# StarrickLiu/StarFlashAttention

Hardware: AMD Instinct MI355X
Metric: attention fwd TFLOPS/GPU (% MFMA peak), bf16 seqlen=4096 hdim=128 (higher is better)
Workload: dtype bf16; 1 GPU; prefill fwd causal, B=16 H=32 S=4096 D=128 per GPU (BASELINE.json configs[2]); batch-sharded, no collectives; global_batch=16, seq_len=4096, heads=32, head_dim=128, causal=True, parallelism=batch-shard x1

## Files before the change

starflashattention_amd/csrc/prefill_w4_kernel.hip:

```cpp
#include "prefill_w4_common.h"

namespace sfa {

namespace {

using namespace prefill;

namespace w4 {
typedef float f32x2 __attribute__((ext_vector_type(2)));

using namespace w4c;

constexpr int kRows = 256;
constexpr int kKeys = 64;
constexpr int kRing = 3;

template <int D> struct Img {
    static constexpr int RG = 512 * (D / 32);
    static constexpr int TILE = 8 * RG;
    static constexpr int K_BASE = 0;
    static constexpr int V_BASE = kRing * TILE;
    static constexpr int Q_BASE = 2 * kRing * TILE;
    static constexpr int TOTAL = Q_BASE + 4 * TILE;
};

#define SFA_AOWN \
    "a0", "a1", "a2", "a3", "a4", "a5", "a6", "a7", "a8", "a9", "a10", "a11", "a12", "a13", "a14", "a15", \
    "a16", "a17", "a18", "a19", "a20", "a21", "a22", "a23", "a24", "a25", "a26", "a27", "a28", "a29", "a30", "a31", \
    "a32", "a33", "a34", "a35", "a36", "a37", "a38", "a39", "a40", "a41", "a42", "a43", "a44", "a45", "a46", "a47", \
    "a48", "a49", "a50", "a51", "a52", "a53", "a54", "a55", "a56", "a57", "a58", "a59", "a60", "a61", "a62", "a63", \
    "a64", "a65", "a66", "a67", "a68", "a69", "a70", "a71", "a72", "a73", "a74", "a75", "a76", "a77", "a78", "a79", \
    "a80", "a81", "a82", "a83", "a84", "a85", "a86", "a87", "a88", "a89", "a90", "a91", "a92", "a93", "a94", "a95", \
    "a96", "a97", "a98", "a99", "a100", "a101", "a102", "a103", "a104", "a105", "a106", "a107", "a108", "a109", "a110", "a111", \
    "a112", "a113", "a114", "a115", "a116", "a117", "a118", "a119", "a120", "a121", "a122", "a123", "a124", "a125", "a126", "a127", \
    "a128", "a129", "a130", "a131", "a132", "a133", "a134", "a135", "a136", "a137", "a138", "a139", "a140", "a141", "a142", "a143", \
    "a144", "a145", "a146", "a147", "a148", "a149", "a150", "a151", "a152", "a153", "a154", "a155", "a156", "a157", "a158", "a159", \
    "a160", "a161", "a162", "a163", "a164", "a165", "a166", "a167", "a168", "a169", "a170", "a171", "a172", "a173", "a174", "a175", \
    "a176", "a177", "a178", "a179", "a180", "a181", "a182", "a183", "a184", "a185", "a186", "a187", "a188", "a189", "a190", "a191"
constexpr int o_reg(int q, int d) { return 16 * (4 * q + d); }
constexpr int q_reg(int q, int ks) { return 128 + 4 * (8 * q + ks); }

template <class Tr, int QB>
__device__ __forceinline__ void own_qk_first(f32x16 &s, typename Tr::mfma_vec k) {
    if constexpr (Tr::id == 1) asm volatile("v_mfma_f32_32x32x16_bf16 %0, %1, a[%c2:%c3], 0" : "=&v"(s) : "v"(k), "n"(QB), "n"(QB + 3) : SFA_AOWN);
    else asm volatile("v_mfma_f32_32x32x16_f16 %0, %1, a[%c2:%c3], 0" : "=&v"(s) : "v"(k), "n"(QB), "n"(QB + 3) : SFA_AOWN);
}
template <class Tr, int QB>
__device__ __forceinline__ void own_qk_first_c(f32x16 &s, typename Tr::mfma_vec k, const f32x16 &c) {
    if constexpr (Tr::id == 1) asm volatile("s_nop 1\n\tv_mfma_f32_32x32x16_bf16 %0, %1, a[%c2:%c3], %4" : "=&v"(s) : "v"(k), "n"(QB), "n"(QB + 3), "v"(c) : SFA_AOWN);
    else asm volatile("s_nop 1\n\tv_mfma_f32_32x32x16_f16 %0, %1, a[%c2:%c3], %4" : "=&v"(s) : "v"(k), "n"(QB), "n"(QB + 3), "v"(c) : SFA_AOWN);
}
template <class Tr, int QB>
__device__ __forceinline__ void own_qk(f32x16 &s, typename Tr::mfma_vec k) {
    if constexpr (Tr::id == 1) asm volatile("v_mfma_f32_32x32x16_bf16 %0, %1, a[%c2:%c3], %0" : "+v"(s) : "v"(k), "n"(QB), "n"(QB + 3) : SFA_AOWN);
    else asm volatile("v_mfma_f32_32x32x16_f16 %0, %1, a[%c2:%c3], %0" : "+v"(s) : "v"(k), "n"(QB), "n"(QB + 3) : SFA_AOWN);
}
template <class Tr, int OB>
__device__ __forceinline__ void own_pv(typename Tr::mfma_vec v, typename Tr::mfma_vec pfrag) {
    if constexpr (Tr::id == 1) asm volatile("v_mfma_f32_32x32x16_bf16 a[%c2:%c3], %0, %1, a[%c2:%c3]" :: "v"(v), "v"(pfrag), "n"(OB), "n"(OB + 15) : SFA_AOWN);
    else asm volatile("v_mfma_f32_32x32x16_f16 a[%c2:%c3], %0, %1, a[%c2:%c3]" :: "v"(v), "v"(pfrag), "n"(OB), "n"(OB + 15) : SFA_AOWN);
}
template <class Tr, int OB>
__device__ __forceinline__ void own_zero(typename Tr::mfma_vec z) {
    if constexpr (Tr::id == 1) asm volatile("s_nop 1\n\tv_mfma_f32_32x32x16_bf16 a[%c1:%c2], %0, %0, 0" :: "v"(z), "n"(OB), "n"(OB + 15) : SFA_AOWN);
    else asm volatile("s_nop 1\n\tv_mfma_f32_32x32x16_f16 a[%c1:%c2], %0, %0, 0" :: "v"(z), "n"(OB), "n"(OB + 15) : SFA_AOWN);
}
__device__ __forceinline__ void own_settle() { asm volatile("s_nop 15\n\ts_nop 15" ::: SFA_AOWN); }
template <int R>
__device__ __forceinline__ float own_read() {
    float x;
    asm volatile("v_accvgpr_read_b32 %0, a%c1" : "=v"(x) : "n"(R) : SFA_AOWN);
    return x;
}
template <int R>
__device__ __forceinline__ void own_scale(float f) {
    float t;
    asm volatile("v_accvgpr_read_b32 %0, a%c2\n\tv_mul_f32 %0, %0, %1\n\tv_accvgpr_write_b32 a%c2, %0" : "=&v"(t) : "v"(f), "n"(R) : SFA_AOWN);
}

template <int D>
struct Acc {
    float msc[2];
    float lsum[2];
    float alpha[2];
    uint32_t pk[2][8];
    f32x16 cinit[2];
};
struct Fin {
    float lsum[2];
    float msc[2];
};

template <int D>
__device__ __forceinline__ void rescale_o(int q, float alpha) {
    own_settle();
    static_for<16 * (D / 32)>([&](auto ic) {
        constexpr int r = decltype(ic)::value;
        if (q == 0) own_scale<o_reg(0, 0) + r>(alpha);
        else own_scale<o_reg(1, 0) + r>(alpha);
    });
    asm volatile("s_nop 1" ::: SFA_AOWN);
}

constexpr int kLead = 8;
constexpr float kNoKey = -1.0e30f;

__device__ __forceinline__ constexpr int el_q(int i) { return (i >> 3) & 1; }
__device__ __forceinline__ constexpr int el_r(int i) { return 8 * (i >> 4) + (i & 7); }

template <class Tr, int ORD, int I>
__device__ __forceinline__ void st_f(f32x16 (&s)[2], const float (&msc)[2], float c2) {
    if constexpr (ORD != 6 && I >= 0 && I < 32)
        asm volatile("v_fma_f32 %0, %0, %1, -%2" : "+v"(s[el_q(I)][el_r(I)]) : "s"(c2), "v"(msc[el_q(I)]));
}
template <int I>
__device__ __forceinline__ void st_x(f32x16 (&s)[2]) {
    if constexpr (I >= 0 && I < 32) asm volatile("v_exp_f32 %0, %0" : "+v"(s[el_q(I)][el_r(I)]));
}
template <class Tr, int I>
__device__ __forceinline__ void st_a(f32x16 (&s)[2], float (&lsum)[2], uint32_t (&pk)[2][8]) {
    if constexpr (I >= 0 && I < 32) {
        constexpr int q = el_q(I), r = el_r(I);
        asm volatile("v_add_f32 %0, %0, %1" : "+v"(lsum[q]) : "v"(s[q][r]));
        if constexpr (I & 1) {
            if constexpr (Tr::id == 1) asm volatile("v_cvt_pk_bf16_f32 %0, %1, %2" : "=v"(pk[q][r >> 1]) : "v"(s[q][r - 1]), "v"(s[q][r]));
            else asm volatile("v_cvt_pk_f16_f32 %0, %1, %2" : "=v"(pk[q][r >> 1]) : "v"(s[q][r - 1]), "v"(s[q][r]));
        }
    }
}
template <class Tr, int D, int ORD>
__device__ __forceinline__ void decide(Acc<D> &acc, int q, f32x16 &s, float mxl, float c2, int &pend) {
    if (ORD == 6) {
        if (__any(mxl > kThr)) {
            const float d = fmaxf(half_max(mxl), 0.f);
            const float al = fast_exp2(-d);
            acc.msc[q] += d;
            acc.lsum[q] *= al;
            acc.alpha[q] = al;
            pend = 1;
#pragma unroll
            for (int r = 0; r < 16; ++r) { s[r] -= d; acc.cinit[q][r] = -acc.msc[q]; }
        }
        return;
    }
    if (__any(__builtin_fmaf(mxl, c2, -kThr) > acc.msc[q])) {
        const float mx = half_max(mxl) * c2;
        const float mnew = fmaxf(acc.msc[q], mx);
        const float al = fast_exp2(acc.msc[q] - mnew);
        acc.msc[q] = mnew;
        acc.lsum[q] *= al;
        acc.alpha[q] = al;
        pend = 1;
    }
}
template <class Tr, int D, int ORD>
__device__ __forceinline__ void fresh_start(Acc<D> &acc, Fin &fin, int q, f32x16 &s, float mxl, float c2) {
    fin.lsum[q] = acc.lsum[q];
    fin.msc[q] = acc.msc[q];
    const float mx = half_max(mxl);
    acc.lsum[q] = 0.f;
    if (ORD == 6) {
        const float m0 = (mx == ninf()) ? 0.f : mx;
        acc.msc[q] = m0;
#pragma unroll
        for (int r = 0; r < 16; ++r) { s[r] -= m0; acc.cinit[q][r] = -m0; }
    } else {
        acc.msc[q] = fmaxf(mx * c2, kNoKey);
    }
}

template <int D>
__device__ __forceinline__ void apply_pending(Acc<D> &acc, int &pend) {
    if (pend) {
#pragma unroll
        for (int q = 0; q < 2; ++q) { rescale_o<D>(q, acc.alpha[q]); acc.alpha[q] = 1.0f; }
        pend = 0;
    }
}

__device__ __forceinline__ int lane_now() {
    int l = __builtin_amdgcn_mbcnt_hi(~0u, __builtin_amdgcn_mbcnt_lo(~0u, 0u));
    asm volatile("" : "+v"(l));
    return l;
}
__device__ __forceinline__ f32x16 mask_tuple(int kbase, int qrow0, int klast) {
    const int l = lane_now();
    const int room = min(klast, qrow0 + (l & 31)) - kbase - 4 * (l >> 5);
    const float ni = ninf();
    float c[16];
    asm volatile(
        "v_cmp_gt_i32_e32 vcc, 0, %16\n\tv_cndmask_b32_e32 %0, 0, %17, vcc\n\t"
        "v_cmp_gt_i32_e32 vcc, 1, %16\n\tv_cndmask_b32_e32 %1, 0, %17, vcc\n\t"
        "v_cmp_gt_i32_e32 vcc, 2, %16\n\tv_cndmask_b32_e32 %2, 0, %17, vcc\n\t"
        "v_cmp_gt_i32_e32 vcc, 3, %16\n\tv_cndmask_b32_e32 %3, 0, %17, vcc\n\t"
        "v_cmp_gt_i32_e32 vcc, 8, %16\n\tv_cndmask_b32_e32 %4, 0, %17, vcc\n\t"
        "v_cmp_gt_i32_e32 vcc, 9, %16\n\tv_cndmask_b32_e32 %5, 0, %17, vcc\n\t"
        "v_cmp_gt_i32_e32 vcc, 10, %16\n\tv_cndmask_b32_e32 %6, 0, %17, vcc\n\t"
        "v_cmp_gt_i32_e32 vcc, 11, %16\n\tv_cndmask_b32_e32 %7, 0, %17, vcc\n\t"
        "v_cmp_gt_i32_e32 vcc, 16, %16\n\tv_cndmask_b32_e32 %8, 0, %17, vcc\n\t"
        "v_cmp_gt_i32_e32 vcc, 17, %16\n\tv_cndmask_b32_e32 %9, 0, %17, vcc\n\t"
        "v_cmp_gt_i32_e32 vcc, 18, %16\n\tv_cndmask_b32_e32 %10, 0, %17, vcc\n\t"
        "v_cmp_gt_i32_e32 vcc, 19, %16\n\tv_cndmask_b32_e32 %11, 0, %17, vcc\n\t"
        "v_cmp_gt_i32_e32 vcc, 24, %16\n\tv_cndmask_b32_e32 %12, 0, %17, vcc\n\t"
        "v_cmp_gt_i32_e32 vcc, 25, %16\n\tv_cndmask_b32_e32 %13, 0, %17, vcc\n\t"
        "v_cmp_gt_i32_e32 vcc, 26, %16\n\tv_cndmask_b32_e32 %14, 0, %17, vcc\n\t"
        "v_cmp_gt_i32_e32 vcc, 27, %16\n\tv_cndmask_b32_e32 %15, 0, %17, vcc"
        : "=&v"(c[0]), "=&v"(c[1]), "=&v"(c[2]), "=&v"(c[3]), "=&v"(c[4]), "=&v"(c[5]), "=&v"(c[6]), "=&v"(c[7]), "=&v"(c[8]),
          "=&v"(c[9]), "=&v"(c[10]), "=&v"(c[11]), "=&v"(c[12]), "=&v"(c[13]), "=&v"(c[14]), "=&v"(c[15])
        : "v"(room), "v"(ni)
        : "vcc");
    f32x16 cm;
#pragma unroll
    for (int r = 0; r < 16; ++r) cm[r] = c[r];
    return cm;
}

template <class Tr, int D, int ORD, int HO, int PH, int NEW, int OLD, int MK, class Hook = NoHook>
__device__ __forceinline__ void hstep(const lds_char *lds, unsigned k_e, unsigned v_e, int vbuf, int kbuf_pref,
                                      f32x16 (&sN)[2], f32x16 (&sO)[2],
                                      Acc<D> &acc, Fin &fin, int &pend, float c2, int mask_n, int kbase_n, int qbase_n,
                                      int klast, const f32x16 &diag0, const f32x16 &ninf16, typename Tr::mfma_vec (&kpre)[D / 16],
                                      const Hook &hook = Hook()) {
    using Vec = typename Tr::mfma_vec;
    constexpr int NKS = D / 16, NDB = D / 32;
    constexpr int RG = Img<D>::RG;
// ... 350 lines not shown
        const unsigned qvoff1 = (unsigned)(qr8 + 8) * rowb + 64u * qsub + 16u * (qslot ^ (2 + (qr8 >> 2)));
        const unsigned long long base = (unsigned long long)(uintptr_t)(a->q + b * a->qs0 + h * a->qs1) + (unsigned long long)row0 * rowb;
        u32x4s srd;
        srd[0] = (unsigned)base;
        srd[1] = (unsigned)(base >> 32) & 0xffffu;
        srd[2] = row0 < a->Sq ? (unsigned)(a->Sq - 1 - row0) * rowb + 2u * D : 0u;
        srd[3] = 0x00020000u;
        const unsigned dst = lds0 + L::Q_BASE + wave * L::TILE;
#pragma unroll
        for (int rg = 0; rg < 8; ++rg)
#pragma unroll
            for (int j = 0; j < NJ; ++j)
                dma_piece(dst + rg * L::RG + 1024 * j, (rg & 1) ? qvoff1 : qvoff0, srd, 128u * j + 16u * (rg >> 1) * rowb);
        young += 8 * NJ;
    };
    auto q_addr = [&](unsigned &qe, unsigned &qo) __attribute__((always_inline)) {
        const int ln = lane_now(), ql31 = ln & 31, qh2 = ln >> 5;
        const unsigned q_e = L::Q_BASE + L::RG * (ql31 >> 3) + 64 * (ql31 & 7) + 16 * (qh2 ^ ((ql31 >> 2) & 3));
        qe = lds0 + q_e + wave * L::TILE;
        qo = lds0 + (q_e ^ 32) + wave * L::TILE;
    };
    auto fetch_q_piece = [&](auto ic, unsigned qe, unsigned qo) __attribute__((always_inline)) {
        constexpr int i = decltype(ic)::value, q = i / NKS, ks = i % NKS;
        const unsigned addr = (ks & 1) ? qo : qe;
        asm volatile("ds_read_b128 a[%c1:%c2], %0 offset:%c3" :: "v"(addr), "n"(q_reg(q, ks)), "n"(q_reg(q, ks) + 3),
                     "n"(4 * L::RG * q + 512 * (ks >> 1)) : SFA_AOWN, "memory");
    };
    auto fetch_q_issue = [&]() __attribute__((always_inline)) {
        asm volatile("s_waitcnt vmcnt(0)" ::: "memory");
        unsigned qe, qo;
        q_addr(qe, qo);
        static_for<NQB * NKS>([&](auto ic) { fetch_q_piece(ic, qe, qo); });
    };
    auto fetch_q_done = [&]() __attribute__((always_inline)) {
        asm volatile("s_waitcnt lgkmcnt(0)" ::: SFA_AOWN, "memory");
        if (PS) {
            static_for<4 * NQB * NKS>([&](auto ic) {
                constexpr int r = 128 + decltype(ic)::value;
                const uint32_t w = bitcast<uint32_t>(own_read<r>());
                const uint32_t w2 = Tr::pack2(Tr::lo_f32(w) * c2, Tr::hi_f32(w) * c2);
                asm volatile("v_accvgpr_write_b32 a%c1, %0" :: "v"(w2), "n"(r) : SFA_AOWN);
            });
            asm volatile("s_nop 1" ::: SFA_AOWN);
        }
    };
    bool qf_on = false;
    bool q_in = false;
    unsigned qf_e = 0, qf_o = 0;
    auto qf_hook = [&](int n) __attribute__((always_inline)) {
        if (n == 15) {
            q_addr(qf_e, qf_o);
            if (qf_on) asm volatile("s_waitcnt vmcnt(8)" ::: "memory");
        }
        static_for<NQB * NKS>([&](auto ic) {
            if (n == 16 + decltype(ic)::value) {
                if (qf_on) fetch_q_piece(ic, qf_e, qf_o);
            }
        });
    };
    auto dma_qf_hook = [&](int n) __attribute__((always_inline)) { dma_hook(n); qf_hook(n); };

    struct ItemW {
        int wq0;
        int qbase;
        int klast;
        int ntw;
        int whole[NQB];
        int t_mask;
        int aligned;
    };
    auto item_w_of = [&](int wv, int coff, int Sk, int qt, int nt, ItemW &w) __attribute__((always_inline)) {
        w.wq0 = qt * kRows + 64 * wv;
        w.qbase = CAUSAL ? w.wq0 + coff : (1 << 29);
        w.klast = Sk - 1;
        w.ntw = nt;
        if (CAUSAL) w.ntw = (w.wq0 + 63 + coff >= 0) ? min(nt, (w.wq0 + 63 + coff) / kKeys + 1) : 0;
#pragma unroll
        for (int q = 0; q < NQB; ++q) w.whole[q] = CAUSAL ? min(w.wq0 + 32 * q + coff - 31, Sk - 32) : Sk - 32;
        const int wmin = min(w.whole[0], w.whole[1]);
        const int jm = wmin < 0 ? 0 : wmin / 32 + 1;
        w.t_mask = max(0, (jm - 1) >> 1);
        const int d0 = w.wq0 + coff;
        w.aligned = CAUSAL && d0 >= 64 && (d0 & 63) == 0 && d0 + 63 <= Sk - 1 && w.ntw == (d0 >> 6) + 1;
    };
    auto mask_bits = [&](const ItemW &w, int kbase) __attribute__((always_inline)) -> int {
        int m = 0;
#pragma unroll
        for (int q = 0; q < NQB; ++q)
            if (kbase > w.whole[q]) m |= 1 << q;
        return m;
    };

    unsigned long long its[5] = {0, 0, 0, 0, 0}, rt0 = 0, rt1 = 0, epi = 0;
    int item_no = 0;
    auto istamp = [&](int which) __attribute__((always_inline)) {
        if constexpr ((DIAG & 256) != 0) {
            if (blockIdx.x == 8) {
                unsigned long long tm, rt;
                asm volatile("s_memtime %0\n\ts_memrealtime %1\n\ts_waitcnt lgkmcnt(0)" : "=s"(tm), "=s"(rt) :: "memory");
                if (which == 0) { its[0] = tm; rt0 = rt; }
                if (which == 1) its[1] = tm;
                if (which == 2) its[2] = tm;
                if (which == 3) its[3] = tm;
                if (which == 4) { its[4] = tm; rt1 = rt; }
                if (which == 5) epi = tm;
                if (which == 6) epi = tm - epi;
            }
        }
    };
    int ev_n = 0;
    auto ev = [&](int kind, int t) __attribute__((always_inline)) {
        if constexpr ((DIAG & 1) != 0) {
            if (blockIdx.x == 8 && item_no < 4 && ev_n < 512) {
                unsigned long long tm;
                asm volatile("s_memtime %0\n\ts_waitcnt lgkmcnt(0)" : "=s"(tm) :: "memory");
                if (lane == 0)
                    reinterpret_cast<unsigned long long *>(arg()->lse)[wave * 512 + ev_n] =
                        (tm & 0xffffffffffffull) | ((unsigned long long)(kind | (t << 4) | (item_no << 12)) << 48);
                ++ev_n;
            }
        }
    };
    auto istore = [&](int ntw, int nt) __attribute__((always_inline)) {
        if constexpr ((DIAG & 1) != 0) ++item_no;
        if constexpr ((DIAG & 256) != 0) {
            if (blockIdx.x == 8 && item_no < 16 && lane == 0) {
                unsigned long long *dst = reinterpret_cast<unsigned long long *>(arg()->lse) + (wave * 16 + item_no) * 8;
                dst[0] = its[0]; dst[1] = its[1]; dst[2] = its[2]; dst[3] = its[3]; dst[4] = its[4];
                dst[5] = (unsigned long long)(unsigned)ntw | ((unsigned long long)(unsigned)nt << 32);
                dst[6] = rt1 - rt0;
                dst[7] = epi;
            }
            ++item_no;
        }
    };

    const f32x16 diag0 = mask_tuple(0, 0, 1 << 29);
    f32x16 ninf16;
#pragma unroll
    for (int r = 0; r < 16; ++r) ninf16[r] = ninf();
    asm volatile("" : "+v"(ninf16));
    {
        const Vec z = bitcast<Vec>(make_uint4(0u, 0u, 0u, 0u));
        static_for<2 * NDB>([&](auto ic) { own_zero<Tr, 16 * decltype(ic)::value>(z); });
    }
    Acc<D> acc;
    Fin fin = {{0.f, 0.f}, {0.f, 0.f}};
    int pend = 0;
    f32x16 sA[NQB], sB[NQB];
    Vec kpre[NKS];
#pragma unroll
    for (int q = 0; q < NQB; ++q) acc.alpha[q] = 1.0f;

    struct EpiArgs { int Sq; uint16_t *obase; long long os2; float *lse_p; long long lse_row0; };
    auto load_epi = [&](int b, int h) __attribute__((always_inline)) -> EpiArgs {
        const ArgPtr a = arg();
        const int Sq = a->Sq;
        return EpiArgs{Sq, a->o + b * a->os0 + h * a->os1, a->os2, a->lse, ((long long)b * a->cur.Hq + h) * Sq};
    };
    auto epilogue_q = [&](const EpiArgs &ea, const ItemW &w, int q, bool have_o) __attribute__((always_inline)) {
        const int Sq = ea.Sq;
        const long long os2 = ea.os2;
        float *const lse_p = ea.lse_p;
        const int ln = lane_now(), l31 = ln & 31, h2 = ln >> 5;
        const int qrow = w.wq0 + 32 * q + l31;
        float ltot = 0.f;
        if (have_o) {
            own_settle();
            ltot = half_sum(fin.lsum[q]);
        }
        const float inv = ltot > 0.f ? 1.0f / ltot : 0.f;
        f32x2 inv2;
        inv2[0] = inv; inv2[1] = inv;
        if (qrow < Sq) {
            uint16_t *orow = ea.obase + (long long)qrow * os2;
            if (have_o) {
                static_for<2 * NDB>([&](auto ic) {
                    constexpr int d = decltype(ic)::value >> 1, g = 2 * (decltype(ic)::value & 1);
                    auto rd2 = [&](auto rc) __attribute__((always_inline)) -> uint32_t {
                        constexpr int r = decltype(rc)::value;
                        f32x2 pr;
                        pr[0] = q == 0 ? own_read<o_reg(0, d) + r>() : own_read<o_reg(1, d) + r>();
                        pr[1] = q == 0 ? own_read<o_reg(0, d) + r + 1>() : own_read<o_reg(1, d) + r + 1>();
                        asm volatile("v_pk_mul_f32 %0, %0, %1" : "+v"(pr) : "v"(inv2));
                        return Tr::pack2(pr[0], pr[1]);
                    };
                    using std::integral_constant;
                    const uint32_t ax = rd2(integral_constant<int, 4 * g + 0>{});
                    const uint32_t ay = rd2(integral_constant<int, 4 * g + 2>{});
                    const uint32_t bx = rd2(integral_constant<int, 4 * g + 4>{});
                    const uint32_t by = rd2(integral_constant<int, 4 * g + 6>{});
                    const auto rx = __builtin_amdgcn_permlane32_swap(ax, bx, false, false);
                    const auto ry = __builtin_amdgcn_permlane32_swap(ay, by, false, false);
                    *reinterpret_cast<uint4 *>(orow + 32 * d + 8 * g + 8 * h2) = make_uint4(rx[0], ry[0], rx[1], ry[1]);
                });
            } else {
#pragma unroll
                for (int d = 0; d < NDB; ++d)
#pragma unroll
                    for (int g = 0; g < 4; g += 2)
                        *reinterpret_cast<uint4 *>(orow + 32 * d + 8 * g + 8 * h2) = make_uint4(0u, 0u, 0u, 0u);
            }
            if (!(DIAG & 257) && lse_p && h2 == 0) {
                const float lse = ltot > 0.f ? (fin.msc[q] + __log2f(ltot)) * kLn2 : ninf();
                lse_p[ea.lse_row0 + qrow] = lse;
            }
        }
        if (have_o) {
            const Vec z = bitcast<Vec>(make_uint4(0u, 0u, 0u, 0u));
            static_for<NDB>([&](auto ic) {
                constexpr int d = decltype(ic)::value;
                if (q == 0) own_zero<Tr, o_reg(0, d)>(z);
                else own_zero<Tr, o_reg(1, d)>(z);
            });
        }
        if (w.wq0 + 32 * q + 31 < Sq) young += 8;
    };
    auto epilogue = [&](int b, int h, const ItemW &w, bool have_o) __attribute__((always_inline)) {
        const EpiArgs ea = load_epi(b, h);
        epilogue_q(ea, w, 0, have_o);
        epilogue_q(ea, w, 1, have_o);
    };
    if (CAUSAL && arg()->cur.coff < 0) {
        W4Cursor c0;
        first_item(c0, false);
        while (c0.live) {
            if (c0.nt == 0) {
                ItemW w0;
                const ArgPtr a0 = arg();
                item_w_of(wave, a0->cur.coff, a0->cur.Sk, c0.qt, 0, w0);
                epilogue(c0.b, c0.h, w0, false);
            }
            next_item(c0, false);
        }
    }
    W4Cursor cc;
    first_item(cc, true);
    if (cc.live) {
        load_q(cc.b, cc.h, cc.qt);
        int pb = 0, ph = 0;
        ItemW pw = {0, 0, 0, 0, {0, 0}, 0, 0};
        bool prev_full = false;
        bool epi_pending = false;
        ItemW cw;
        bool full_wave;
        for (;;) {
            {
                const ArgPtr a = arg();
                item_w_of(wave, a->cur.coff, a->cur.Sk, cc.qt, cc.nt, cw);
            }
            istamp(0);
            if (!q_in) fetch_q_issue();
            fetch_q_done();
            q_in = false;
            ev(5, 0);
            wait_and_sync();
            ev(2, 63);
            istamp(1);
            {
                const int k1 = ring_next(kcur);
                if (prev_full) {
                    hstep<Tr, D, ORD, 1, 1, 2, 1, 1>(lds, k_e, v_e, vcur, k1, sA, sB, acc, fin, pend, c2,
                                                          mask_bits(cw, 0), 0, cw.qbase, cw.klast, diag0, ninf16, kpre, dma_hook);
                    istamp(5);
                    ev(3, 63);
                    epilogue(pb, ph, pw, true);
                    ev(4, 63);
                    istamp(6);
                } else {
                    const lds_char *const kb_e = lds + (k_e + k1), *const kb_o = lds + ((k_e ^ 32) + k1);
#pragma unroll
                    for (int i = 0; i < NKS; ++i)
                        kpre[i] = bitcast<Vec>(lds_read16(((i & 1) ? kb_o : kb_e) + 512 * (i >> 1)));
                    hstep<Tr, D, ORD, 1, 1, 2, 0, 1>(lds, k_e, v_e, vcur, k1, sA, sB, acc, fin, pend, c2,
                                                          mask_bits(cw, 0), 0, cw.qbase, cw.klast, diag0, ninf16, kpre, dma_hook);
                    ev(3, 63);
                    if (epi_pending) { epilogue_q(load_epi(pb, ph), pw, 1, true); epi_pending = false; ev(4, 63); }
                }
                kcur = k1;
                vcur = ring_next(vcur);
            }

            istamp(2);
            const int nt = cc.nt, ntw = cw.ntw;
            const int b = cc.b, h = cc.h;
            W4Cursor nx = cc;
            next_item(nx, true);
            const bool chained = nx.live != 0;
            const int qreq_t = chained ? max(nt - 3, -1) : -2;
            if (qreq_t == -1) load_q(nx.b, nx.h, nx.qt);
            const bool qf_ok = qreq_t >= 0;
            if (ntw == 0) epilogue(b, h, cw, false);

            full_wave = !CAUSAL || ntw == nt;
            int t = 0;
            auto step_done = [&]() __attribute__((always_inline)) {
                if (t == qreq_t) load_q(nx.b, nx.h, nx.qt);
                kcur = ring_next(kcur);
                vcur = ring_next(vcur);
                ++t;
            };
            {
                const int t_inner = min(ntw - 1, cw.t_mask);
                while (t < t_inner) {
                    const int k1 = ring_next(kcur);
                    hstep<Tr, D, ORD, 0, 0, 1, 1, 0>(lds, k_e, v_e, vcur, k1, sB, sA, acc, fin, pend, c2,
                                                          0, 0, 0, 0, diag0, ninf16, kpre);
                    ev(1, t);
                    wait_and_sync();
                    ev(2, t);
                    hstep<Tr, D, ORD, 1, 1, 1, 1, 0>(lds, k_e, v_e, vcur, k1, sA, sB, acc, fin, pend, c2,
                                                          0, 0, 0, 0, diag0, ninf16, kpre, dma_hook);
                    ev(3, t);
                    step_done();
                }
            }
            istamp(3);
            if (ntw > 0) {
                if (!PS && cw.aligned) {
                    {
                        const int k1 = ring_next(kcur);
                        hstep<Tr, D, ORD, 0, 0, 1, 1, 0>(lds, k_e, v_e, vcur, k1, sB, sA, acc, fin, pend, c2,
                                                          0, 0, 0, 0, diag0, ninf16, kpre);
                        ev(1, t);
                        wait_and_sync();
                        ev(2, t);
                        hstep<Tr, D, ORD, 1, 1, 1, 1, PS ? 1 : 2>(lds, k_e, v_e, vcur, k1, sA, sB, acc, fin, pend, c2,
                                                                   1, t * kKeys + 64, cw.qbase, cw.klast, diag0, ninf16, kpre, dma_hook);
                        ev(3, t);
                        step_done();
                    }
                    qf_on = qf_ok && ntw == nt;
                    hstep<Tr, D, ORD, 0, 0, 1, 1, PS ? 1 : 3>(lds, k_e, v_e, vcur, ring_next(kcur), sB, sA, acc, fin, pend, c2,
                                                               3, t * kKeys + 32, cw.qbase, cw.klast, diag0, ninf16, kpre, qf_hook);
                    if (qf_on) { q_in = true; qf_on = false; }
                    ev(1, t);
                } else {
                    for (;;) {
                        const int k1 = ring_next(kcur);
                        const int kbase = t * kKeys;
                        qf_on = qf_ok && ntw == nt && t + 1 == nt;
                        hstep<Tr, D, ORD, 0, 0, 1, 1, 1>(lds, k_e, v_e, vcur, k1, sB, sA, acc, fin, pend, c2,
                                                          mask_bits(cw, kbase + 32), kbase + 32, cw.qbase, cw.klast, diag0, ninf16, kpre, qf_hook);
                        if (qf_on) { q_in = true; qf_on = false; }
                        ev(1, t);
                        if (t + 1 == ntw) break;
                        wait_and_sync();
                        ev(2, t);
                        hstep<Tr, D, ORD, 1, 1, 1, 1, 1>(lds, k_e, v_e, vcur, k1, sA, sB, acc, fin, pend, c2,
                                                          mask_bits(cw, kbase + 64), kbase + 64, cw.qbase, cw.klast, diag0, ninf16, kpre, dma_hook);
                        ev(3, t);
                        step_done();
                    }
                }
                if (!full_wave) {
                    wait_and_sync();
                    ev(2, t);
                    qf_on = qf_ok && ntw + 1 == nt;
                    hstep<Tr, D, ORD, 1, 1, 0, 1, 1>(lds, k_e, v_e, vcur, ring_next(kcur), sA, sB, acc, fin, pend, c2,
                                                         0, 0, cw.qbase, cw.klast, diag0, ninf16, kpre, dma_qf_hook);
                    if (qf_on) { q_in = true; qf_on = false; }
                    ev(3, t);
                    epilogue_q(load_epi(b, h), cw, 0, true);
                    ev(4, t);
                    epi_pending = true;
                    step_done();
                }
            }
            if (!full_wave) {
                while (t + 1 < nt) {
                    wait_and_sync();
                    ev(2, t);
                    produce_v();
                    produce_k();
                    ev(3, t);
                    if (epi_pending) { epilogue_q(load_epi(b, h), cw, 1, true); epi_pending = false; ev(4, t); }
                    if (qf_ok && t == nt - 2) { fetch_q_issue(); q_in = true; }
                    step_done();
                }
            }
            istamp(4);
            istore(ntw, nt);
            if (!chained) break;
            prev_full = full_wave;
            pb = b; ph = h; pw = cw;
            cc = nx;
        }
        wait_and_sync();
        if (full_wave) {
            hstep<Tr, D, ORD, 1, 1, 0, 1, 1>(lds, k_e, v_e, vcur, ring_next(kcur), sA, sB, acc, fin, pend, c2,
                                                  0, 0, cw.qbase, cw.klast, diag0, ninf16, kpre, dma_hook);
            epilogue(cc.b, cc.h, cw, true);
        } else if (epi_pending) {
            epilogue_q(load_epi(cc.b, cc.h), cw, 1, true);
        }
    }
    asm volatile("s_waitcnt vmcnt(0)" ::: "memory");
}

template <class Tr, int D, int ORD, int DIAG = 0>
int launch_w4_t(const PrefillKernelParams &p, bool causal, hipStream_t stream) {
    using namespace w4;
    const int lds = Img<D>::TOTAL;
    const int nq = (p.Sq + kRows - 1) / kRows;
    const int U = causal ? (nq + 1) / 2 : nq;
    const long long units_xcd = (long long)p.bh_per_xcd * U;
    const int nslots = (int)(units_xcd < 32 ? units_xcd : 32);
    W4Args a;
    a.q = p.q; a.o = p.o; a.lse = p.lse;
    a.qs0 = p.qs[0]; a.qs1 = p.qs[1]; a.os0 = p.os[0]; a.os1 = p.os[1]; a.os2 = p.os[2];
    a.q_rowb = (unsigned)(2 * p.qs[2]);
    a.Sq = p.Sq;
    a.c2 = p.scale_log2;
    a.kv.k = p.k; a.kv.v = p.v;
    a.kv.ks0 = p.ks[0]; a.kv.ks1 = p.ks[1]; a.kv.vs0 = p.vs[0]; a.kv.vs1 = p.vs[1];
    a.kv.k_rowb = (unsigned)(2 * p.ks[2]); a.kv.v_rowb = (unsigned)(2 * p.vs[2]);
    a.kv.k_extent = (int)((long long)(p.Sk - 1) * a.kv.k_rowb + 2 * D);
    a.kv.v_extent = (int)((long long)(p.Sk - 1) * a.kv.v_rowb + 2 * D);
    a.cur.U = U; a.cur.Hq = p.Hq; a.cur.bh_per_xcd = p.bh_per_xcd; a.cur.BH = p.B * p.Hq; a.cur.nq = nq;
    a.cur.Sk = p.Sk; a.cur.coff = p.Sk - p.Sq; a.cur.G = p.Hq / p.Hkv;
    a.cur.adv_hl = nslots / U; a.cur.adv_i = nslots - a.cur.adv_hl * U;
    a.cur.adv_b = a.cur.adv_hl / p.Hq; a.cur.adv_h = a.cur.adv_hl - a.cur.adv_b * p.Hq;
    dim3 grid(8u * nslots), block(kThreadsW4);
    static DynLdsAttr attr_c, attr_f;
    if (const int rc = causal ? attr_c.ensure(reinterpret_cast<const void *>(&prefill_w4_kernel<Tr, D, true, ORD, DIAG>), lds, "prefill_w4_kernel")
                              : attr_f.ensure(reinterpret_cast<const void *>(&prefill_w4_kernel<Tr, D, false, ORD, DIAG>), lds, "prefill_w4_kernel"))
        return rc;
    if (causal) hipLaunchKernelGGL((prefill_w4_kernel<Tr, D, true, ORD, DIAG>), grid, block, lds, stream, a);
    else hipLaunchKernelGGL((prefill_w4_kernel<Tr, D, false, ORD, DIAG>), grid, block, lds, stream, a);
    return check_launch("prefill_w4_kernel");
}

}

#ifdef SFA_W4_PART
#if SFA_W4_PART == 1
int launch_prefill_w4_fp16_exact(const PrefillKernelParams &p, bool causal, hipStream_t stream) { return launch_w4_t<Fp16, 128, 2>(p, causal, stream); }
#elif SFA_W4_PART == 2
int launch_prefill_w4_fp16_prescaled(const PrefillKernelParams &p, bool causal, hipStream_t stream) { return launch_w4_t<Fp16, 128, 6>(p, causal, stream); }
#elif SFA_W4_PART == 3
int launch_prefill_w4_bf16_prescaled(const PrefillKernelParams &p, bool causal, hipStream_t stream) { return launch_w4_t<Bf16, 128, 6>(p, causal, stream); }
#else
#error "SFA_W4_PART is 1, 2 or 3"
#endif
#else

bool prefill_w4_serves(const PrefillKernelParams &p, int head_dim) {
    if (head_dim != 128) return false;
    const long long k_ext = (long long)(p.Sk - 1) * 2 * p.ks[2] + 2 * head_dim, v_ext = (long long)(p.Sk - 1) * 2 * p.vs[2] + 2 * head_dim;
    const long long q_ext = (long long)(p.Sq - 1) * 2 * p.qs[2] + 2 * head_dim;
    return k_ext < (1ll << 31) && v_ext < (1ll << 31) && q_ext < (1ll << 31) && p.ks[2] * 2 < (1ll << 24) && p.vs[2] * 2 < (1ll << 24) &&
           p.qs[2] * 2 < (1ll << 24);
}

int launch_prefill_w4(const PrefillKernelParams &p, int dtype, int head_dim, bool causal, hipStream_t stream, int force) {
    if (dtype != SFA_DTYPE_FP16 && dtype != SFA_DTYPE_BF16)
        return fail(SFA_ERR_BAD_DTYPE, "sfa_prefill_fwd: dtype %d is not fp16(0)/bf16(1)", dtype);
    if (head_dim != 128)
        return fail(SFA_ERR_UNSUPPORTED_HEAD_DIM, "sfa_prefill_fwd: the 4-wave kernel serves head_dim 128 (got %d)", head_dim);
    if (!prefill_w4_serves(p, head_dim))
        return fail(SFA_ERR_BAD_SHAPE, "sfa_prefill_fwd: one head's Q/K/V rows span more than 2 GiB");
    const bool prescaled = force == 0 ? p.fast_scale != 0 : force == 1;
#ifdef SFA_WITH_VARIANTS
    if (force == 3) return launch_w4_t<Bf16, 128, 2, 256>(p, causal, stream);
    if (force == 4) return launch_w4_t<Bf16, 128, 2, 1>(p, causal, stream);
#endif
#ifdef SFA_W4_DEV
    if (dtype != SFA_DTYPE_BF16 || prescaled)
        return fail(SFA_ERR_BAD_DTYPE, "sfa_prefill_fwd: this SFA_W4_DEV build of the 4-wave kernel serves bf16 exact scale only");
    return launch_w4_t<Bf16, 128, 2>(p, causal, stream);
#else
    if (dtype == SFA_DTYPE_FP16)
        return prescaled ? launch_prefill_w4_fp16_prescaled(p, causal, stream) : launch_prefill_w4_fp16_exact(p, causal, stream);
    return prescaled ? launch_prefill_w4_bf16_prescaled(p, causal, stream) : launch_w4_t<Bf16, 128, 2>(p, causal, stream);
#endif
}
#endif

}
```

Measured before the change: 1058 TFLOPS.

## Software-pipeline epilogue accumulator reads and hoist output pointer setup

Restructures the attention epilogue so accumulator register reads for the next group are issued in the same asm block as the scaling of the current group, which lets the read latency overlap with the multiplies. Output and LSE pointer arithmetic moves earlier and is forced into scalar registers, so it stays off the critical path after the final MMA. Row normalisation and LSE values for both query blocks are computed before a single settle wait. The no-key zero-fill path is split into its own function. This adds register pressure and hand-scheduled asm that the compiler can no longer reorder.

Result: no change. 1061 TFLOPS (median of 6 runs) (+0.3%).

```diff
diff --git a/starflashattention_amd/csrc/prefill_w4_kernel.hip b/starflashattention_amd/csrc/prefill_w4_kernel.hip
--- a/starflashattention_amd/csrc/prefill_w4_kernel.hip
+++ b/starflashattention_amd/csrc/prefill_w4_kernel.hip
@@ -71,6 +71,30 @@
     float x;
     asm volatile("v_accvgpr_read_b32 %0, a%c1" : "=v"(x) : "n"(R) : SFA_AOWN);
     return x;
+}
+template <int R>
+__device__ __forceinline__ void own_group_first(f32x2 (&r)[4]) {
+    asm volatile("v_accvgpr_read_b32 %0, a%c8\n\tv_accvgpr_read_b32 %1, a%c9\n\t"
+                 "v_accvgpr_read_b32 %2, a%c10\n\tv_accvgpr_read_b32 %3, a%c11\n\t"
+                 "v_accvgpr_read_b32 %4, a%c12\n\tv_accvgpr_read_b32 %5, a%c13\n\t"
+                 "v_accvgpr_read_b32 %6, a%c14\n\tv_accvgpr_read_b32 %7, a%c15"
+                 : "=v"(r[0][0]), "=v"(r[0][1]), "=v"(r[1][0]), "=v"(r[1][1]), "=v"(r[2][0]), "=v"(r[2][1]), "=v"(r[3][0]), "=v"(r[3][1])
+                 : "n"(R), "n"(R + 1), "n"(R + 2), "n"(R + 3), "n"(R + 4), "n"(R + 5), "n"(R + 6), "n"(R + 7) : SFA_AOWN);
+}
+template <int R>
+__device__ __forceinline__ void own_group(f32x2 (&m)[4], f32x2 inv2, f32x2 (&r)[4]) {
+    asm volatile("v_pk_mul_f32 %0, %0, %12\n\tv_pk_mul_f32 %1, %1, %12\n\tv_pk_mul_f32 %2, %2, %12\n\tv_pk_mul_f32 %3, %3, %12\n\t"
+                 "v_accvgpr_read_b32 %4, a%c13\n\tv_accvgpr_read_b32 %5, a%c14\n\t"
+                 "v_accvgpr_read_b32 %6, a%c15\n\tv_accvgpr_read_b32 %7, a%c16\n\t"
+                 "v_accvgpr_read_b32 %8, a%c17\n\tv_accvgpr_read_b32 %9, a%c18\n\t"
+                 "v_accvgpr_read_b32 %10, a%c19\n\tv_accvgpr_read_b32 %11, a%c20"
+                 : "+v"(m[0]), "+v"(m[1]), "+v"(m[2]), "+v"(m[3]),
+                   "=&v"(r[0][0]), "=&v"(r[0][1]), "=&v"(r[1][0]), "=&v"(r[1][1]), "=&v"(r[2][0]), "=&v"(r[2][1]), "=&v"(r[3][0]), "=&v"(r[3][1])
+                 : "v"(inv2), "n"(R), "n"(R + 1), "n"(R + 2), "n"(R + 3), "n"(R + 4), "n"(R + 5), "n"(R + 6), "n"(R + 7) : SFA_AOWN);
+}
+__device__ __forceinline__ void own_group_last(f32x2 (&m)[4], f32x2 inv2) {
+    asm volatile("v_pk_mul_f32 %0, %0, %4\n\tv_pk_mul_f32 %1, %1, %4\n\tv_pk_mul_f32 %2, %2, %4\n\tv_pk_mul_f32 %3, %3, %4"
+                 : "+v"(m[0]), "+v"(m[1]), "+v"(m[2]), "+v"(m[3]) : "v"(inv2) : SFA_AOWN);
 }
 template <int R>
 __device__ __forceinline__ void own_scale(float f) {
@@ -727,74 +751,93 @@
 #pragma unroll
     for (int q = 0; q < NQB; ++q) acc.alpha[q] = 1.0f;
 
-    struct EpiArgs { int Sq; uint16_t *obase; long long os2; float *lse_p; long long lse_row0; };
+    struct EpiArgs { int Sq; uint16_t *obase; long long os2; float *lse_row; };
+    auto load_epi_at = [&](ArgPtr a, int b, int h, int &x0, int &x1) __attribute__((always_inline)) -> EpiArgs {
+        int Sq = a->Sq, Hq = a->cur.Hq;
+        uint16_t *o = a->o;
+        float *lp = a->lse;
+        long long os0 = a->os0, os1 = a->os1, os2 = a->os2;
+        asm volatile("" : "+s"(Sq), "+s"(Hq), "+s"(o), "+s"(lp), "+s"(os0), "+s"(os1), "+s"(os2), "+s"(x0), "+s"(x1));
+        float *const lrow = lp + ((long long)b * Hq + h) * Sq;
+        EpiArgs ea{Sq, o + b * os0 + h * os1, os2, lp ? lrow : lp};
+        asm volatile("" : "+s"(ea.Sq), "+s"(ea.obase), "+s"(ea.os2), "+s"(ea.lse_row));
+        return ea;
+    };
     auto load_epi = [&](int b, int h) __attribute__((always_inline)) -> EpiArgs {
-        const ArgPtr a = arg();
-        const int Sq = a->Sq;
-        return EpiArgs{Sq, a->o + b * a->os0 + h * a->os1, a->os2, a->lse, ((long long)b * a->cur.Hq + h) * Sq};
-    };
-    auto epilogue_q = [&](const EpiArgs &ea, const ItemW &w, int q, bool have_o) __attribute__((always_inline)) {
-        const int Sq = ea.Sq;
-        const long long os2 = ea.os2;
-        float *const lse_p = ea.lse_p;
+        int x0 = 0, x1 = 0;
+        return load_epi_at(arg(), b, h, x0, x1);
+    };
+    typedef uint32_t u32x4 __attribute__((ext_vector_type(4)));
+    typedef u32x4 __attribute__((address_space(1))) *GlobalU4;
+    typedef float __attribute__((address_space(1))) *GlobalF32;
+    struct EpiRow { f32x2 inv2; float lse; uint16_t *orow; int qrow; };
+    auto epi_row = [&](const EpiArgs &ea, const ItemW &w, int q) __attribute__((always_inline)) -> EpiRow {
         const int ln = lane_now(), l31 = ln & 31, h2 = ln >> 5;
-        const int qrow = w.wq0 + 32 * q + l31;
-        float ltot = 0.f;
-        if (have_o) {
-            own_settle();
-            ltot = half_sum(fin.lsum[q]);
-        }
+        EpiRow r;
+        r.qrow = w.wq0 + 32 * q + l31;
+        const float ltot = half_sum(fin.lsum[q]);
         const float inv = ltot > 0.f ? 1.0f / ltot : 0.f;
-        f32x2 inv2;
-        inv2[0] = inv; inv2[1] = inv;
-        if (qrow < Sq) {
-            uint16_t *orow = ea.obase + (long long)qrow * os2;
-            if (have_o) {
-                static_for<2 * NDB>([&](auto ic) {
-                    constexpr int d = decltype(ic)::value >> 1, g = 2 * (decltype(ic)::value & 1);
-                    auto rd2 = [&](auto rc) __attribute__((always_inline)) -> uint32_t {
-                        constexpr int r = decltype(rc)::value;
-                        f32x2 pr;
-                        pr[0] = q == 0 ? own_read<o_reg(0, d) + r>() : own_read<o_reg(1, d) + r>();
-                        pr[1] = q == 0 ? own_read<o_reg(0, d) + r + 1>() : own_read<o_reg(1, d) + r + 1>();
-                        asm volatile("v_pk_mul_f32 %0, %0, %1" : "+v"(pr) : "v"(inv2));
-                        return Tr::pack2(pr[0], pr[1]);
-                    };
-                    using std::integral_constant;
-                    const uint32_t ax = rd2(integral_constant<int, 4 * g + 0>{});
-                    const uint32_t ay = rd2(integral_constant<int, 4 * g + 2>{});
-                    const uint32_t bx = rd2(integral_constant<int, 4 * g + 4>{});
-                    const uint32_t by = rd2(integral_constant<int, 4 * g + 6>{});
-                    const auto rx = __builtin_amdgcn_permlane32_swap(ax, bx, false, false);
-                    const auto ry = __builtin_amdgcn_permlane32_swap(ay, by, false, false);
-                    *reinterpret_cast<uint4 *>(orow + 32 * d + 8 * g + 8 * h2) = make_uint4(rx[0], ry[0], rx[1], ry[1]);
-                });
-            } else {
+        r.inv2[0] = inv; r.inv2[1] = inv;
+        r.lse = ltot > 0.f ? (fin.msc[q] + __log2f(ltot)) * kLn2 : ninf();
+        r.orow = ea.obase + (long long)r.qrow * ea.os2 + 8 * h2;
+        asm volatile("" : "+v"(r.inv2), "+v"(r.lse), "+v"(r.orow));
+        return r;
+    };
+    auto epi_store = [&](const EpiArgs &ea, const EpiRow &er, const ItemW &w, auto qc) __attribute__((always_inline)) {
+        constexpr int q = decltype(qc)::value, NG = 2 * NDB;
+        if (er.qrow < ea.Sq) {
+            f32x2 pa[4], pb[4];
+            own_group_first<o_reg(q, 0)>(pa);
+            static_for<NG>([&](auto ic) {
+                constexpr int i = decltype(ic)::value;
+                f32x2 (&m)[4] = (i & 1) ? pb : pa;
+                f32x2 (&r)[4] = (i & 1) ? pa : pb;
+                if constexpr (i + 1 < NG) own_group<o_reg(q, 0) + 8 * (i + 1)>(m, er.inv2, r);
+                else own_group_last(m, er.inv2);
+                const uint32_t ax = Tr::pack2(m[0][0], m[0][1]), ay = Tr::pack2(m[1][0], m[1][1]);
+                const uint32_t bx = Tr::pack2(m[2][0], m[2][1]), by = Tr::pack2(m[3][0], m[3][1]);
+                const auto rx = __builtin_amdgcn_permlane32_swap(ax, bx, false, false);
+                const auto ry = __builtin_amdgcn_permlane32_swap(ay, by, false, false);
+                *(GlobalU4)(er.orow + 16 * i) = u32x4{rx[0], ry[0], rx[1], ry[1]};
+            });
+            if (!(DIAG & 257) && ea.lse_row && lane_now() < 32) ((GlobalF32)ea.lse_row)[er.qrow] = er.lse;
+        }
+        {
+            const Vec z = bitcast<Vec>(make_uint4(0u, 0u, 0u, 0u));
+            static_for<NDB>([&](auto ic) { own_zero<Tr, o_reg(q, decltype(ic)::value)>(z); });
+        }
+        if (w.wq0 + 32 * q + 31 < ea.Sq) young += 8;
+    };
+    constexpr std::integral_constant<int, 0> QB0{};
+    constexpr std::integral_constant<int, 1> QB1{};
+    auto epilogue_q = [&](const EpiArgs &ea, const ItemW &w, auto qc) __attribute__((always_inline)) {
+        const EpiRow er = epi_row(ea, w, decltype(qc)::value);
+        own_settle();
+        epi_store(ea, er, w, qc);
+    };
+    auto epilogue = [&](const EpiArgs &ea, const ItemW &w) __attribute__((always_inline)) {
+        const EpiRow e0 = epi_row(ea, w, 0), e1 = epi_row(ea, w, 1);
+        own_settle();
+        epi_store(ea, e0, w, QB0);
+        epi_store(ea, e1, w, QB1);
+    };
+    auto epilogue_nokey = [&](int b, int h, const ItemW &w) __attribute__((always_inline)) {
+        const EpiArgs ea = load_epi(b, h);
+        const int ln = lane_now(), l31 = ln & 31, h2 = ln >> 5;
+#pragma unroll
+        for (int q = 0; q < NQB; ++q) {
+            const int qrow = w.wq0 + 32 * q + l31;
+            if (qrow < ea.Sq) {
+                uint16_t *orow = ea.obase + (long long)qrow * ea.os2;
 #pragma unroll
                 for (int d = 0; d < NDB; ++d)
 #pragma unroll
                     for (int g = 0; g < 4; g += 2)
-                        *reinterpret_cast<uint4 *>(orow + 32 * d + 8 * g + 8 * h2) = make_uint4(0u, 0u, 0u, 0u);
-            }
-            if (!(DIAG & 257) && lse_p && h2 == 0) {
-                const float lse = ltot > 0.f ? (fin.msc[q] + __log2f(ltot)) * kLn2 : ninf();
-                lse_p[ea.lse_row0 + qrow] = lse;
-            }
-        }
-        if (have_o) {
-            const Vec z = bitcast<Vec>(make_uint4(0u, 0u, 0u, 0u));
-            static_for<NDB>([&](auto ic) {
-                constexpr int d = decltype(ic)::value;
-                if (q == 0) own_zero<Tr, o_reg(0, d)>(z);
-                else own_zero<Tr, o_reg(1, d)>(z);
-            });
-        }
-        if (w.wq0 + 32 * q + 31 < Sq) young += 8;
-    };
-    auto epilogue = [&](int b, int h, const ItemW &w, bool have_o) __attribute__((always_inline)) {
-        const EpiArgs ea = load_epi(b, h);
-        epilogue_q(ea, w, 0, have_o);
-        epilogue_q(ea, w, 1, have_o);
+                        *(GlobalU4)(orow + 32 * d + 8 * g + 8 * h2) = u32x4{0u, 0u, 0u, 0u};
+                if (!(DIAG & 257) && ea.lse_row && h2 == 0) ((GlobalF32)ea.lse_row)[qrow] = ninf();
+            }
+            if (w.wq0 + 32 * q + 31 < ea.Sq) young += 8;
+        }
     };
     if (CAUSAL && arg()->cur.coff < 0) {
         W4Cursor c0;
@@ -804,7 +847,7 @@
                 ItemW w0;
                 const ArgPtr a0 = arg();
                 item_w_of(wave, a0->cur.coff, a0->cur.Sk, c0.qt, 0, w0);
-                epilogue(c0.b, c0.h, w0, false);
+                epilogue_nokey(c0.b, c0.h, w0);
             }
             next_item(c0, false);
         }
@@ -820,9 +863,12 @@
         ItemW cw;
         bool full_wave;
         for (;;) {
+            EpiArgs pea;
             {
                 const ArgPtr a = arg();
-                item_w_of(wave, a->cur.coff, a->cur.Sk, cc.qt, cc.nt, cw);
+                int coff = a->cur.coff, Sk = a->cur.Sk;
+                pea = load_epi_at(a, pb, ph, coff, Sk);
+                item_w_of(wave, coff, Sk, cc.qt, cc.nt, cw);
             }
             istamp(0);
             if (!q_in) fetch_q_issue();
@@ -839,7 +885,7 @@
                                                           mask_bits(cw, 0), 0, cw.qbase, cw.klast, diag0, ninf16, kpre, dma_hook);
                     istamp(5);
                     ev(3, 63);
-                    epilogue(pb, ph, pw, true);
+                    epilogue(pea, pw);
                     ev(4, 63);
                     istamp(6);
                 } else {
@@ -850,7 +896,7 @@
                     hstep<Tr, D, ORD, 1, 1, 2, 0, 1>(lds, k_e, v_e, vcur, k1, sA, sB, acc, fin, pend, c2,
                                                           mask_bits(cw, 0), 0, cw.qbase, cw.klast, diag0, ninf16, kpre, dma_hook);
                     ev(3, 63);
-                    if (epi_pending) { epilogue_q(load_epi(pb, ph), pw, 1, true); epi_pending = false; ev(4, 63); }
+                    if (epi_pending) { epilogue_q(pea, pw, QB1); epi_pending = false; ev(4, 63); }
                 }
                 kcur = k1;
                 vcur = ring_next(vcur);
@@ -865,7 +911,8 @@
             const int qreq_t = chained ? max(nt - 3, -1) : -2;
             if (qreq_t == -1) load_q(nx.b, nx.h, nx.qt);
             const bool qf_ok = qreq_t >= 0;
-            if (ntw == 0) epilogue(b, h, cw, false);
+            if (ntw == 0) epilogue_nokey(b, h, cw);
+            EpiArgs cea = pea;
 
             full_wave = !CAUSAL || ntw == nt;
             int t = 0;
@@ -936,7 +983,8 @@
                                                          0, 0, cw.qbase, cw.klast, diag0, ninf16, kpre, dma_qf_hook);
                     if (qf_on) { q_in = true; qf_on = false; }
                     ev(3, t);
-                    epilogue_q(load_epi(b, h), cw, 0, true);
+                    cea = load_epi(b, h);
+                    epilogue_q(cea, cw, QB0);
                     ev(4, t);
                     epi_pending = true;
                     step_done();
@@ -949,7 +997,7 @@
                     produce_v();
                     produce_k();
                     ev(3, t);
-                    if (epi_pending) { epilogue_q(load_epi(b, h), cw, 1, true); epi_pending = false; ev(4, t); }
+                    if (epi_pending) { epilogue_q(cea, cw, QB1); epi_pending = false; ev(4, t); }
                     if (qf_ok && t == nt - 2) { fetch_q_issue(); q_in = true; }
                     step_done();
                 }
@@ -961,13 +1009,14 @@
             pb = b; ph = h; pw = cw;
             cc = nx;
         }
+        const EpiArgs lea = load_epi(cc.b, cc.h);
         wait_and_sync();
         if (full_wave) {
             hstep<Tr, D, ORD, 1, 1, 0, 1, 1>(lds, k_e, v_e, vcur, ring_next(kcur), sA, sB, acc, fin, pend, c2,
                                                   0, 0, cw.qbase, cw.klast, diag0, ninf16, kpre, dma_hook);
-            epilogue(cc.b, cc.h, cw, true);
+            epilogue(lea, cw);
         } else if (epi_pending) {
-            epilogue_q(load_epi(cc.b, cc.h), cw, 1, true);
+            epilogue_q(lea, cw, QB1);
         }
     }
     asm volatile("s_waitcnt vmcnt(0)" ::: "memory");
```
